# SeanNaren/deepspeech.pytorch

Hardware: NVIDIA H100
Metric: utterances/sec (train step, 161x1000 spectrogram) (higher is better)
Workload: dtype fp16-operands(rnn)+tf32(conv/fc)

## Files before the change

deepspeech.pytorch_b200/csrc/conv_tc.cu:

```cuda
#include "common.cuh"
#include "tc_common.cuh"

namespace ds2 {
int make_tmap_4d_f32(CUtensorMap* out, const float* base, const unsigned long long dims[4],
                     const unsigned long long strides_bytes[3], const unsigned int box[4]);
int make_tmap_nd_f32(CUtensorMap* out, const float* base, int rank, const unsigned long long* dims,
                     const unsigned long long* strides_bytes, const unsigned int* box);

namespace cv {
constexpr int CH = 32, KW = 11, NN = KW * CH;
constexpr int MP = 64, TO = MP - (KW - 1);
constexpr int A_BYTES = MP * 128;
constexpr int W_HALF = (NN / 2) * 128;
constexpr int STAGE_BYTES = A_BYTES + 2 * W_HALF;
constexpr int STAGES = 3;
constexpr int OUT_LD = 33, OUT_FLOATS = TO * OUT_LD;
constexpr int THREADS = 384;
constexpr int PRODUCER_REGS = 40, MMA_REGS = 232;
constexpr int ORDER_BAR = 1, EPI_BAR = 3;
constexpr int SMEM_BYTES = 1024 + STAGES * STAGE_BYTES + 2 * OUT_FLOATS * 4 + 256;
}

__device__ __forceinline__ void tma_load_4d_w(void* dst, const CUtensorMap* m, uint64_t* bar, int c0, int c1, int c2,
                                              int c3) {
  asm volatile(
      "{\n\t.reg .pred pe;\n\telect.sync _|pe, 0xffffffff;\n\t"
      "@pe cp.async.bulk.tensor.4d.shared::cluster.global.tile.mbarrier::complete_tx::bytes [%0], [%1, {%3, %4, %5, %6}], [%2];\n\t}"
      ::"r"(tc::smem_u32(dst)), "l"(reinterpret_cast<uint64_t>(m)), "r"(tc::smem_u32(bar)), "r"(c0), "r"(c1), "r"(c2),
        "r"(c3)
      : "memory");
}
__device__ __forceinline__ void tma_load_5d_w(void* dst, const CUtensorMap* m, uint64_t* bar, int c0, int c1, int c2,
                                              int c3, int c4) {
  asm volatile(
      "{\n\t.reg .pred pe;\n\telect.sync _|pe, 0xffffffff;\n\t"
      "@pe cp.async.bulk.tensor.5d.shared::cluster.global.tile.mbarrier::complete_tx::bytes [%0], [%1, {%3, %4, %5, %6, %7}], [%2];\n\t}"
      ::"r"(tc::smem_u32(dst)), "l"(reinterpret_cast<uint64_t>(m)), "r"(tc::smem_u32(bar)), "r"(c0), "r"(c1), "r"(c2),
        "r"(c3), "r"(c4)
      : "memory");
}

struct ConvTcParams {
  CUtensorMap tmA;
  CUtensorMap tmW;
  int B, T, R_in;
  int ntt;
  ConvRows rows[2];
  int tiles0, tiles;
  int row_mul, row_step, w_step, out_row_mul;
  float* out;
  size_t ob, oc, orow;
  const float* bias;
  const int32_t* out_len;
  double* stat_sums;
  double* piv_sums;
};

struct ConvTile {
  int t0, d, b, cls, j_lo, nj;
};
__device__ __forceinline__ ConvTile conv_tile(const ConvTcParams& p, int u) {
  ConvTile t;
  t.cls = u >= p.tiles0;
  if (t.cls) u -= p.tiles0;
  const ConvRows& rc = p.rows[t.cls];
  t.t0 = (u % p.ntt) * cv::TO;
  u /= p.ntt;
  t.d = u % rc.R_out;
  t.b = u / rc.R_out;
  int j_lo = 0, j_hi = rc.J;
  const int r0 = p.row_mul * t.d + rc.row_off;
  while (j_lo < j_hi && (r0 + j_lo * p.row_step < 0 || r0 + j_lo * p.row_step >= p.R_in)) ++j_lo;
  while (j_hi > j_lo && (r0 + (j_hi - 1) * p.row_step < 0 || r0 + (j_hi - 1) * p.row_step >= p.R_in)) --j_hi;
  t.j_lo = j_lo;
  t.nj = j_hi - j_lo;
  return t;
}

__device__ __forceinline__ void named_bar_sync(int id, int threads) {
  asm volatile("bar.sync %0, %1;" ::"r"(id), "r"(threads) : "memory");
}
__device__ __forceinline__ void named_bar_arrive(int id, int threads) {
  asm volatile("bar.arrive %0, %1;" ::"r"(id), "r"(threads) : "memory");
}

__global__ void __launch_bounds__(cv::THREADS, 1) conv_tc_kernel(const __grid_constant__ ConvTcParams p) {
  using namespace cv;
  using namespace tc;
  extern __shared__ uint8_t smem_raw[];
  uint8_t* smem = reinterpret_cast<uint8_t*>((reinterpret_cast<uintptr_t>(smem_raw) + 1023) & ~(uintptr_t)1023);
  float* out_s0 = reinterpret_cast<float*>(smem + STAGES * STAGE_BYTES);
  uint64_t* full = reinterpret_cast<uint64_t*>(out_s0 + 2 * OUT_FLOATS);
  uint64_t* empty = full + STAGES;

  const int warp = threadIdx.x / 32, lane = threadIdx.x % 32;

  if (warp == 0 && lane == 0) {
    tma_prefetch_desc(&p.tmA);
    tma_prefetch_desc(&p.tmW);
    for (int i = 0; i < STAGES; ++i) { mbar_init(&full[i], 1); mbar_init(&empty[i], 1); }
    fence_barrier_init();
  }
  __syncthreads();

  if (warp < 4) {
    setmaxnreg_dec<PRODUCER_REGS>();
    if (warp == 0) {
      int g = 0;
      for (int u = blockIdx.x; u < p.tiles; u += gridDim.x) {
        const ConvTile t = conv_tile(p, u);
        const ConvRows& rc = p.rows[t.cls];
        for (int jj = 0; jj < t.nj; ++jj, ++g) {
          const int j = t.j_lo + jj;
          const int r = p.row_mul * t.d + rc.row_off + j * p.row_step;
          const int wi = rc.w_off + j * p.w_step;
          const int s = g % STAGES;
          mbar_wait(&empty[s], ((g / STAGES) & 1) ^ 1);
          mbar_arrive_expect_tx_w(&full[s], (uint32_t)STAGE_BYTES);
          uint8_t* st = smem + s * STAGE_BYTES;
          tma_load_4d_w(st, &p.tmA, &full[s], 0, t.t0 - 5, r, t.b);
          tma_load_3d_w(st + A_BYTES, &p.tmW, &full[s], 0, 0, wi);
          tma_load_3d_w(st + A_BYTES + W_HALF, &p.tmW, &full[s], 0, NN / 2, wi);
        }
      }
    }
    return;
  }

  setmaxnreg_inc<MMA_REGS>();
  const int wg = warp / 4 - 1, w = warp % 4;
  const bool leader = (threadIdx.x & 127) == 0;
  float* out_s = out_s0 + wg * OUT_FLOATS;
  int g = 0;
  int i = 0;
  for (int u = blockIdx.x; u < p.tiles; u += gridDim.x, ++i) {
    const ConvTile t = conv_tile(p, u);
    if ((i & 1) != wg) {
      g += t.nj;
      continue;
    }
    if (i > 0) named_bar_sync(ORDER_BAR + wg, 256);
    float acc[NN / 2];
#pragma unroll
    for (int k = 0; k < NN / 2; ++k) acc[k] = 0.f;
    for (int jj = 0; jj < t.nj; ++jj, ++g) {
      const int s = g % STAGES;
      mbar_wait(&full[s], (g / STAGES) & 1);
      const uint64_t ad = smem_desc_sw128(smem_u32(smem + s * STAGE_BYTES));
      const uint64_t bd = smem_desc_sw128(smem_u32(smem + s * STAGE_BYTES + A_BYTES));
      wg_fence();
#pragma unroll
      for (int k = 0; k < 4; ++k) {
#pragma unroll
        for (int h = 0; h < 2; ++h)
          Wgmma<NN / 2, false>::mma(acc + (NN / 4) * h, ad + (uint64_t)(2 * k),
                                    bd + (uint64_t)(W_HALF / 16 * h + 2 * k), 1u);
      }
      wg_commit();
      wg_wait<1>();
      if (jj > 0 && leader) mbar_arrive(&empty[(g - 1) % STAGES]);
    }
    if (u + (int)gridDim.x < p.tiles) named_bar_arrive(ORDER_BAR + (wg ^ 1), 256);
    wg_wait<0>();
    if (t.nj > 0 && leader) mbar_arrive(&empty[(g - 1) % STAGES]);

    named_bar_sync(EPI_BAR + wg, 128);
#pragma unroll
    for (int kw = 0; kw < KW; ++kw) {
#pragma unroll
      for (int ib = 4 * kw; ib < 4 * kw + 4; ++ib) {
#pragma unroll
        for (int e = 0; e < 4; ++e) {
          const int pl = 16 * w + (lane >> 2) + 8 * (e >> 1);
          const int co = 8 * (ib % 4) + 2 * (lane & 3) + (e & 1);
          const int to = pl - kw;
          if (to >= 0 && to < TO) {
            float* o = out_s + to * OUT_LD + co;
            *o = (kw == 0 ? 0.f : *o) + acc[4 * ib + e];
          }
        }
      }
      named_bar_sync(EPI_BAR + wg, 128);
    }

    const int L = p.out_len ? p.out_len[t.b] : p.T;
    const int orow_idx = p.out_row_mul * t.d + p.rows[t.cls].out_row_off;
    for (int cc = 0; cc < 8; ++cc) {
      const int c = w * 8 + cc;
      const float bv = p.bias ? p.bias[c] : 0.f;
      float* op = p.out + (size_t)t.b * p.ob + (size_t)c * p.oc + (size_t)orow_idx * p.orow;
      float s1 = 0.f, s2 = 0.f, e1 = 0.f, e2 = 0.f;
      for (int to = lane; to < TO; to += 32) {
        const int tt = t.t0 + to;
        if (tt < p.T) {
          const float val = (tt < L) ? out_s[to * OUT_LD + c] + bv : 0.f;
          op[tt] = val;
          s1 += val;
          s2 = fmaf(val, val, s2);
          const float dv = val - bv;
          e1 += dv;
          e2 = fmaf(dv, dv, e2);
        }
      }
      if (p.stat_sums) {
        s1 = warp_sum(s1);
        s2 = warp_sum(s2);
        if (lane == 0) {
          atomicAdd(&p.stat_sums[c], (double)s1);
          atomicAdd(&p.stat_sums[CH + c], (double)s2);
        }
      }
      if (p.piv_sums) {
        e1 = warp_sum(e1);
        e2 = warp_sum(e2);
        if (lane == 0) {
          atomicAdd(&p.piv_sums[c], (double)e1);
          atomicAdd(&p.piv_sums[CH + c], (double)e2);
        }
      }
    }
  }
}

__global__ void pack_conv2_tc_fwd_kernel(const float* __restrict__ w2, float* __restrict__ wn) {
  int i = blockIdx.x * blockDim.x + threadIdx.x, n = 21 * cv::NN * 32;
  if (i >= n) return;
  int ci = i % 32, nn = (i / 32) % cv::NN, kh = i / (32 * cv::NN);
  int kw = nn / 32, co = nn % 32;
  wn[i] = w2[(((size_t)co * 32 + ci) * 21 + kh) * 11 + kw];
}
__global__ void pack_conv2_tc_bwd_kernel(const float* __restrict__ w2, float* __restrict__ wd) {
  int i = blockIdx.x * blockDim.x + threadIdx.x, n = 21 * cv::NN * 32;
  if (i >= n) return;
  int co = i % 32, nn = (i / 32) % cv::NN, kh = i / (32 * cv::NN);
  int kwi = nn / 32, ci = nn % 32;
  wd[i] = w2[(((size_t)co * 32 + ci) * 21 + kh) * 11 + (10 - kwi)];
}

__global__ void nchw_to_cl_kernel(int R, int T, const float* __restrict__ in, float* __restrict__ out) {
  __shared__ float tile[32][33];
  const int b = blockIdx.z, r = blockIdx.y, t0 = blockIdx.x * 32;
  for (int c = threadIdx.y; c < 32; c += 8) {
    int t = t0 + threadIdx.x;
    tile[c][threadIdx.x] = (t < T) ? in[(((size_t)b * 32 + c) * R + r) * T + t] : 0.f;
  }
  __syncthreads();
  for (int j = threadIdx.y; j < 32; j += 8) {
    int t = t0 + j;
    if (t < T) out[(((size_t)b * R + r) * T + t) * 32 + threadIdx.x] = tile[threadIdx.x][j];
  }
}

int nchw_to_cl(int B, int R, int T, const float* in, float* out, cudaStream_t st) {
  DS2_LAUNCH(nchw_to_cl_kernel, dim3(cdiv(T, 32), R, B), dim3(32, 8), 0, st, R, T, in, out);
  return DS2_OK;
}

int pack_conv2_tc(const float* w2, float* wn_fwd, float* wd_bwd, cudaStream_t st) {
  const int n = 21 * cv::NN * 32;
  if (wn_fwd) DS2_LAUNCH(pack_conv2_tc_fwd_kernel, cdiv(n, 256), 256, 0, st, w2, wn_fwd);
  if (wd_bwd) DS2_LAUNCH(pack_conv2_tc_bwd_kernel, cdiv(n, 256), 256, 0, st, w2, wd_bwd);
  return DS2_OK;
}

static int make_tmap_cl(CUtensorMap* out, const float* base, int T, int R, int B);

int conv_tc_run(const float* in_cl, int B, int T, int R_in, const float* taps, int n_taps, int row_mul, int row_step,
                int w_step, int out_row_mul, const ConvRows* rows, int n_classes, float* out, size_t ob, size_t oc,
                size_t orow, const float* bias, const int32_t* out_len, double* stat_sums, double* piv_sums,
                cudaStream_t st) {
  ConvTcParams p{};
  int rc = make_tmap_cl(&p.tmA, in_cl, T, R_in, B);
  if (rc) return rc;
  rc = make_tmap_3d(&p.tmW, taps, 32, cv::NN, n_taps, 32, (size_t)32 * cv::NN, 32, cv::NN / 2, 1);
  if (rc) return rc;
  p.B = B; p.T = T; p.R_in = R_in; p.ntt = cdiv(T, cv::TO);
  p.tiles = 0;
  for (int c = 0; c < n_classes; ++c) {
    p.rows[c] = rows[c];
    p.tiles += p.ntt * rows[c].R_out * B;
    if (c == 0) p.tiles0 = p.tiles;
  }
  p.row_mul = row_mul; p.row_step = row_step; p.w_step = w_step; p.out_row_mul = out_row_mul;
  p.out = out; p.ob = ob; p.oc = oc; p.orow = orow;
  p.bias = bias; p.out_len = out_len; p.stat_sums = stat_sums; p.piv_sums = piv_sums;
  static DeviceOnce attr_once;
  if (attr_once.first()) {
    DS2_CHECK_CUDA(cudaFuncSetAttribute(conv_tc_kernel, cudaFuncAttributeMaxDynamicSharedMemorySize, cv::SMEM_BYTES));
    attr_once.done();
  }
  const int grid = p.tiles < device_sm_count() ? p.tiles : device_sm_count();
  DS2_LAUNCH(conv_tc_kernel, grid, cv::THREADS, cv::SMEM_BYTES, st, p);
  return DS2_OK;
}

namespace wg {
constexpr int KT = 32;
constexpr int KH = 21;
constexpr int KH_PER = 2;
constexpr int GROUPS = 6;
constexpr int A_BYTES = KH_PER * 32 * 128;
constexpr int B_BYTES = cv::NN * 128;
constexpr int STAGE_BYTES = A_BYTES + B_BYTES;
constexpr int STAGES = 3;
constexpr int THREADS = 384;
constexpr int SMEM_BYTES = 1024 + STAGES * STAGE_BYTES + 256;
}

struct WgradParams {
  CUtensorMap tmDz;
  CUtensorMap tmS4;
  CUtensorMap tmS2;
  CUtensorMap tmS1;
  int B, T, slices;
  float* part;
};
__constant__ int KW_OF_BLOCK[11] = {1, 0, 5, 4, 3, 2, 9, 8, 7, 6, 10};

__global__ void shift_copies_kernel(size_t rows, int T, const float* __restrict__ a1, float* __restrict__ a1r) {
  const int Tp = T + 4;
  size_t i = (size_t)blockIdx.x * blockDim.x + threadIdx.x, n = rows * Tp, stride = (size_t)gridDim.x * blockDim.x;
  for (; i < n; i += stride) {
    const int t = (int)(i % Tp);
    const float* src = a1 + (i / Tp) * T;
#pragma unroll
    for (int sft = 0; sft <= 3; ++sft) {
      const int ts = t - sft;
      a1r[(size_t)sft * n + i] = (ts >= 0 && ts < T) ? src[ts] : 0.f;
    }
  }
}

__global__ void __launch_bounds__(wg::THREADS, 1) conv2_wgrad_tc_kernel(const __grid_constant__ WgradParams p) {
  using namespace wg;
  using namespace tc;
  extern __shared__ uint8_t smem_raw[];
  uint8_t* smem = reinterpret_cast<uint8_t*>((reinterpret_cast<uintptr_t>(smem_raw) + 1023) & ~(uintptr_t)1023);
  uint64_t* full = reinterpret_cast<uint64_t*>(smem + STAGES * STAGE_BYTES);
  uint64_t* empty = full + STAGES;
  const int warp = threadIdx.x / 32, lane = threadIdx.x % 32;
  const int parity = blockIdx.x / GROUPS, kh0 = parity + 2 * KH_PER * (blockIdx.x % GROUPS);
  if (kh0 >= KH) return;
  const int nkh = min(KH_PER, (KH - 1 - kh0) / 2 + 1);
  const int nr = (DS2_CONV1_D - parity + 1) / 2;
  const int pairs = p.B * nr;
  const int per = (pairs + (int)gridDim.y - 1) / (int)gridDim.y;
  const int p0 = blockIdx.y * per, p1 = min(pairs, p0 + per);
  const int nkt = (p.T + KT - 1) / KT;
  auto row_active = [&](int r) {
    const int d_hi = (r + 10 - kh0) / 2, d_lo = (r + 10 - (kh0 + 2 * (nkh - 1))) / 2;
    return d_hi >= 0 && d_lo < DS2_CONV2_D;
  };

  if (warp == 0 && lane == 0) {
    tma_prefetch_desc(&p.tmDz);
    tma_prefetch_desc(&p.tmS4);
    for (int i = 0; i < STAGES; ++i) { mbar_init(&full[i], 1); mbar_init(&empty[i], 2); }
    fence_barrier_init();
  }
  __syncthreads();

  int nchunks = 0;
  for (int pi = p0; pi < p1; ++pi)
    if (row_active(2 * (pi % nr) + parity)) nchunks += nkt;

  if (warp == 0) {
    int s = 0;
    uint32_t ph = 0;
    for (int pi = p0; pi < p1; ++pi) {
      const int b = pi / nr, r = 2 * (pi % nr) + parity;
      if (!row_active(r)) continue;
      for (int kt = 0; kt < nkt; ++kt) {
        mbar_wait(&empty[s], ph ^ 1);
        mbar_arrive_expect_tx_w(&full[s], (uint32_t)(nkh * 32 * 128 + cv::NN * 128));
        uint8_t* st = smem + s * STAGE_BYTES;
        for (int i = 0; i < nkh; ++i)
          tma_load_4d_w(st + i * 4096, &p.tmDz, &full[s], kt * KT, (r + 10 - kh0) / 2 - i, 0, b);
        uint8_t* nb = st + A_BYTES;
        tma_load_5d_w(nb, &p.tmS2, &full[s], kt * KT - 4, r, 0, b, 0);
        tma_load_5d_w(nb + 2 * 4096, &p.tmS4, &full[s], kt * KT, r, 0, b, 0);
        tma_load_5d_w(nb + 6 * 4096, &p.tmS4, &full[s], kt * KT + 4, r, 0, b, 0);
        tma_load_5d_w(nb + 10 * 4096, &p.tmS1, &full[s], kt * KT + 8, r, 0, b, 3);
        if (++s == STAGES) { s = 0; ph ^= 1; }
      }
    }
  } else if (warp >= 4) {
    const int wg = warp / 4 - 1;
    float acc[cv::NN / 4];
#pragma unroll
    for (int i = 0; i < cv::NN / 4; ++i) acc[i] = 0.f;
    int s = 0;
    uint32_t ph = 0;
    for (int c = 0; c < nchunks; ++c) {
      mbar_wait(&full[s], ph);
      const uint64_t ad = smem_desc_sw128(smem_u32(smem + s * STAGE_BYTES));
      const uint64_t bd = smem_desc_sw128(smem_u32(smem + s * STAGE_BYTES + A_BYTES + wg * cv::W_HALF));
      wg_fence();
#pragma unroll
      for (int k = 0; k < 4; ++k) Wgmma<cv::NN / 2, false>::mma(acc, ad + (uint64_t)(2 * k), bd + (uint64_t)(2 * k), 1u);
      wg_release(&empty[s]);
      if (++s == STAGES) { s = 0; ph ^= 1; }
    }
    const int w = warp % 4;
    float* tile = p.part + ((size_t)blockIdx.x * gridDim.y + blockIdx.y) * 64 * cv::NN;
#pragma unroll
    for (int i = 0; i < cv::NN / 16; ++i) {
#pragma unroll
      for (int hh = 0; hh < 2; ++hh) {
        const int m = 16 * w + (lane >> 2) + 8 * hh;
        const int n = cv::NN / 2 * wg + 8 * i + 2 * (lane & 3);
        *reinterpret_cast<float2*>(tile + (size_t)m * cv::NN + n) = make_float2(acc[4 * i + 2 * hh], acc[4 * i + 2 * hh + 1]);
      }
    }
  }
}

__global__ void conv2_wgrad_reduce_kernel(int slices, const float* __restrict__ part, float* __restrict__ dw2) {
  using namespace wg;
  const int idx = blockIdx.x * blockDim.x + threadIdx.x;
  if (idx >= 32 * 32 * KH * cv::KW) return;
  const int kw = idx % cv::KW, kh = (idx / cv::KW) % KH, ci = (idx / (cv::KW * KH)) % 32, co = idx / (cv::KW * KH * 32);
  const int parity = kh & 1, q = (kh - parity) / 2, x = parity * GROUPS + q / KH_PER, m = 32 * (q % KH_PER) + co;
  int blk = 0;
  while (KW_OF_BLOCK[blk] != kw) ++blk;
  const float* src = part + (size_t)x * slices * 64 * cv::NN + (size_t)m * cv::NN + blk * 32 + ci;
  float s = 0.f;
  for (int y = 0; y < slices; ++y) s += src[(size_t)y * 64 * cv::NN];
  dw2[idx] = s;
}

int conv2_wgrad_tc(const float* dz2, const float* a1, float* a1_shifted , float* part,
                   int B, int T, float* dw2, cudaStream_t st) {
  if (T % 4 != 0) return 1;
  WgradParams p{};
  {
    const size_t rows = (size_t)B * 32 * 81;
    DS2_LAUNCH(shift_copies_kernel, device_sm_count() * 8, 256, 0, st, rows, T, a1, a1_shifted);
    const unsigned long long Tq = (unsigned long long)T + 4;
    unsigned long long dims[5] = {Tq, 81ull, 32ull, (unsigned long long)B, 4ull};
    unsigned long long str[4] = {Tq * 4, 81ull * Tq * 4, 32ull * 81 * Tq * 4, (unsigned long long)rows * Tq * 4};
    unsigned int box[5] = {32u, 1u, 32u, 1u, 4u};
    int rc = make_tmap_nd_f32(&p.tmS4, a1_shifted, 5, dims, str, box);
    if (rc) return rc;
    box[4] = 2u;
    rc = make_tmap_nd_f32(&p.tmS2, a1_shifted, 5, dims, str, box);
    if (rc) return rc;
    box[4] = 1u;
    rc = make_tmap_nd_f32(&p.tmS1, a1_shifted, 5, dims, str, box);
    if (rc) return rc;
  }
  {
    unsigned long long dims[4] = {(unsigned long long)T, 41ull, 32ull, (unsigned long long)B};
    unsigned long long str[3] = {(unsigned long long)T * 4, (unsigned long long)41 * T * 4, (unsigned long long)32 * 41 * T * 4};
    unsigned int box[4] = {32u, 1u, 32u, 1u};
    int rc = make_tmap_4d_f32(&p.tmDz, dz2, dims, str, box);
    if (rc) return rc;
  }
  p.B = B; p.T = T; p.slices = 12; p.part = part;
  static DeviceOnce attr_once;
  if (attr_once.first()) {
    DS2_CHECK_CUDA(cudaFuncSetAttribute(conv2_wgrad_tc_kernel, cudaFuncAttributeMaxDynamicSharedMemorySize, wg::SMEM_BYTES));
    attr_once.done();
  }
  DS2_LAUNCH(conv2_wgrad_tc_kernel, dim3(2 * wg::GROUPS, p.slices), wg::THREADS, wg::SMEM_BYTES, st, p);
  DS2_LAUNCH(conv2_wgrad_reduce_kernel, cdiv(32 * 32 * wg::KH * cv::KW, 256), 256, 0, st, p.slices, part, dw2);
  return DS2_OK;
}

namespace w1 {
constexpr int KT = 32;
constexpr int DI = 4, RJ = 8;
constexpr int NROWS = 12 * RJ;
constexpr int CLASSES = 6;
constexpr int A_BYTES = 32 * DI * 128;
constexpr int B_BYTES = NROWS * 128;
constexpr int STAGE_BYTES = A_BYTES + B_BYTES;
constexpr int STAGES = 6;
constexpr int THREADS = 384;
constexpr int SMEM_BYTES = 1024 + STAGES * STAGE_BYTES + 256;
}
__constant__ int KW1_OF_GROUP[12] = {5, 6, 3, 4, 1, 2, -1, 0, 9, 10, 7, 8};

struct Wgrad1Params {
  CUtensorMap tmDz;
  CUtensorMap tmX8;
  CUtensorMap tmX4;
  int B, Tp;
  float* part;
};

__global__ void conv1_shift_copies_kernel(int B, int T, int Tp, const float* __restrict__ x, float* __restrict__ xs) {
  const int U = Tp + 4;
  const size_t rows = (size_t)B * DS2_NUM_FREQ, n = rows * U, total = 8 * n;
  for (size_t i = (size_t)blockIdx.x * blockDim.x + threadIdx.x; i < total; i += (size_t)gridDim.x * blockDim.x) {
    const int up = (int)(i % U);
    const size_t row = (i / U) % rows;
    const int sq = (int)(i / n), q = sq & 1, sft = sq >> 1;
    const int u = up - sft, tx = 2 * u + q;
    xs[i] = (u >= 0 && tx < T) ? x[row * T + tx] : 0.f;
  }
}

__global__ void __launch_bounds__(w1::THREADS, 1) conv1_wgrad_tc_kernel(const __grid_constant__ Wgrad1Params p) {
  using namespace w1;
  using namespace tc;
  extern __shared__ uint8_t smem_raw[];
  uint8_t* smem = reinterpret_cast<uint8_t*>((reinterpret_cast<uintptr_t>(smem_raw) + 1023) & ~(uintptr_t)1023);
  uint64_t* full = reinterpret_cast<uint64_t*>(smem + STAGES * STAGE_BYTES);
  uint64_t* empty = full + STAGES;
  const int warp = threadIdx.x / 32, lane = threadIdx.x % 32;
  const int cls = blockIdx.x;
  const int ndb = (DS2_CONV1_D + DI - 1) / DI;
  const int pairs = p.B * ndb;
  const int per = (pairs + (int)gridDim.y - 1) / (int)gridDim.y;
  const int p0 = blockIdx.y * per, p1 = min(pairs, p0 + per);
  const int nkt = (p.Tp + KT - 1) / KT;
  auto block_active = [&](int db) {
    const int r0 = 2 * DI * db - 20 + RJ * cls;
    return r0 + RJ - 1 >= 0 && r0 < DS2_NUM_FREQ;
  };

  if (warp == 0 && lane == 0) {
    tma_prefetch_desc(&p.tmDz);
    tma_prefetch_desc(&p.tmX8);
    tma_prefetch_desc(&p.tmX4);
    for (int i = 0; i < STAGES; ++i) { mbar_init(&full[i], 1); mbar_init(&empty[i], 2); }
    fence_barrier_init();
  }
  __syncthreads();

  int nchunks = 0;
  for (int pi = p0; pi < p1; ++pi)
    if (block_active(pi % ndb)) nchunks += nkt;

  if (warp == 0) {
    int s = 0;
    uint32_t ph = 0;
    for (int pi = p0; pi < p1; ++pi) {
      const int b = pi / ndb, db = pi % ndb;
      if (!block_active(db)) continue;
      const int d0 = DI * db, r0 = 2 * d0 - 20 + RJ * cls;
      for (int kt = 0; kt < nkt; ++kt) {
        mbar_wait(&empty[s], ph ^ 1);
        mbar_arrive_expect_tx_w(&full[s], (uint32_t)STAGE_BYTES);
        uint8_t* st = smem + s * STAGE_BYTES;
        tma_load_4d_w(st, &p.tmDz, &full[s], kt * KT, d0, 0, b);
        tma_load_5d_w(st + A_BYTES, &p.tmX8, &full[s], kt * KT, r0, b, 0, 0);
        tma_load_5d_w(st + A_BYTES + 64 * 128, &p.tmX4, &full[s], kt * KT + 4, r0, b, 0, 2);
        if (++s == STAGES) { s = 0; ph ^= 1; }
      }
    }
  } else if (warp >= 4) {
    const int wg = warp / 4 - 1;
    float acc[NROWS / 2];
#pragma unroll
    for (int i = 0; i < NROWS / 2; ++i) acc[i] = 0.f;
    int s = 0;
    uint32_t ph = 0;
    for (int c = 0; c < nchunks; ++c) {
      mbar_wait(&full[s], ph);
      const uint64_t ad = smem_desc_sw128(smem_u32(smem + s * STAGE_BYTES)) + (uint64_t)(512 * wg);
      const uint64_t bd = smem_desc_sw128(smem_u32(smem + s * STAGE_BYTES + A_BYTES));
      wg_fence();
#pragma unroll
      for (int k = 0; k < 4; ++k) Wgmma<NROWS, false>::mma(acc, ad + (uint64_t)(2 * k), bd + (uint64_t)(2 * k), 1u);
      wg_release(&empty[s]);
      if (++s == STAGES) { s = 0; ph ^= 1; }
    }
    const int w = warp % 4;
    float* tile = p.part + ((size_t)cls * gridDim.y + blockIdx.y) * 128 * NROWS;
#pragma unroll
    for (int i = 0; i < NROWS / 8; ++i) {
#pragma unroll
      for (int hh = 0; hh < 2; ++hh) {
        const int m = 64 * wg + 16 * w + (lane >> 2) + 8 * hh, n = 8 * i + 2 * (lane & 3);
        *reinterpret_cast<float2*>(tile + (size_t)m * NROWS + n) = make_float2(acc[4 * i + 2 * hh], acc[4 * i + 2 * hh + 1]);
      }
    }
  }
}

__global__ void conv1_wgrad_reduce_kernel(int slices, const float* __restrict__ part, float* __restrict__ dw1) {
  using namespace w1;
  const int idx = blockIdx.x * blockDim.x + threadIdx.x;
  if (idx >= 32 * 41 * 11) return;
  const int kw = idx % 11, kh = (idx / 11) % 41, co = idx / (11 * 41);
  int grp = 0;
  while (KW1_OF_GROUP[grp] != kw) ++grp;
  float s = 0.f;
  for (int cls = 0; cls < CLASSES; ++cls)
    for (int i = 0; i < DI; ++i) {
      const int j = kh - RJ * cls + 2 * i;
      if (j < 0 || j >= RJ) continue;
      const float* src = part + (size_t)cls * slices * 128 * NROWS + (size_t)(DI * co + i) * NROWS + grp * RJ + j;
      for (int y = 0; y < slices; ++y) s += src[(size_t)y * 128 * NROWS];
    }
  dw1[idx] = s;
}

size_t conv_wgrad_tc_partial_floats() {
  const size_t c2 = (size_t)2 * wg::GROUPS * 12 * 64 * cv::NN, c1 = (size_t)w1::CLASSES * 24 * 128 * w1::NROWS;
  return c2 > c1 ? c2 : c1;
}

int conv1_wgrad_tc(const float* dz1, const float* x, float* xs, float* part, int B, int T, int Tp, float* dw1,
                   cudaStream_t st) {
  if (Tp % 4 != 0) return 1;
  Wgrad1Params p{};
  const unsigned long long U = (unsigned long long)Tp + 4, F = DS2_NUM_FREQ;
  DS2_LAUNCH(conv1_shift_copies_kernel, device_sm_count() * 8, 256, 0, st, B, T, Tp, x, xs);
  {
    unsigned long long dims[5] = {U, F, (unsigned long long)B, 2ull, 4ull};
    unsigned long long str[4] = {U * 4, F * U * 4, (unsigned long long)B * F * U * 4, 2ull * B * F * U * 4};
    unsigned int box[5] = {32u, (unsigned int)w1::RJ, 1u, 2u, 4u};
    int rc = make_tmap_nd_f32(&p.tmX8, xs, 5, dims, str, box);
    if (rc) return rc;
    box[4] = 2u;
    rc = make_tmap_nd_f32(&p.tmX4, xs, 5, dims, str, box);
    if (rc) return rc;
  }
  {
    unsigned long long dims[4] = {(unsigned long long)Tp, (unsigned long long)DS2_CONV1_D, 32ull, (unsigned long long)B};
    unsigned long long str[3] = {(unsigned long long)Tp * 4, (unsigned long long)DS2_CONV1_D * Tp * 4,
                                 32ull * DS2_CONV1_D * Tp * 4};
    unsigned int box[4] = {32u, (unsigned int)w1::DI, 32u, 1u};
    int rc = make_tmap_4d_f32(&p.tmDz, dz1, dims, str, box);
    if (rc) return rc;
  }
  p.B = B; p.Tp = Tp; p.part = part;
  static DeviceOnce attr_once;
  if (attr_once.first()) {
    DS2_CHECK_CUDA(cudaFuncSetAttribute(conv1_wgrad_tc_kernel, cudaFuncAttributeMaxDynamicSharedMemorySize, w1::SMEM_BYTES));
    attr_once.done();
  }
  DS2_LAUNCH(conv1_wgrad_tc_kernel, dim3(w1::CLASSES, 24), w1::THREADS, w1::SMEM_BYTES, st, p);
  DS2_LAUNCH(conv1_wgrad_reduce_kernel, cdiv(32 * 41 * 11, 256), 256, 0, st, 24, part, dw1);
  return DS2_OK;
}

}

namespace ds2 {
int make_tmap_4d_f32(CUtensorMap* out, const float* base, const unsigned long long dims[4],
                     const unsigned long long strides_bytes[3], const unsigned int box[4]);
static int make_tmap_cl(CUtensorMap* out, const float* base, int T, int R, int B) {
  unsigned long long dims[4] = {32ull, (unsigned long long)T, (unsigned long long)R, (unsigned long long)B};
  unsigned long long str[3] = {128ull, (unsigned long long)T * 128ull, (unsigned long long)R * T * 128ull};
  unsigned int box[4] = {32u, (unsigned int)cv::MP, 1u, 1u};
  return make_tmap_4d_f32(out, base, dims, str, box);
}
}
```

Baseline: 655.4.

## Widen conv weight-gradient tiles and pipeline wgmma commits with deferred stage release

The conv2 weight-gradient kernel now covers four kernel-height taps per block instead of two, halving the group count. Each consumer warpgroup takes its own 64-row half of A and computes both N halves, with producer/consumer register rebalancing. The conv1 weight-gradient kernel processes two frequency classes per block, sharing the dz tile across both and halving its grid. Both kernels commit wgmma groups asynchronously and release the previous stage only after wait<1>, so MMAs overlap the next barrier wait. The cost is fewer blocks, which lowers SM occupancy, plus larger accumulators and more register pressure.

```diff
diff --git a/deepspeech.pytorch_b200/csrc/conv_tc.cu b/deepspeech.pytorch_b200/csrc/conv_tc.cu
--- a/deepspeech.pytorch_b200/csrc/conv_tc.cu
+++ b/deepspeech.pytorch_b200/csrc/conv_tc.cu
@@ -297,14 +297,17 @@
 namespace wg {
 constexpr int KT = 32;
 constexpr int KH = 21;
-constexpr int KH_PER = 2;
-constexpr int GROUPS = 6;
-constexpr int A_BYTES = KH_PER * 32 * 128;
+constexpr int KH_PER = 4;
+constexpr int GROUPS = 3;
+constexpr int M = KH_PER * 32;
+constexpr int A_BYTES = M * 128;
 constexpr int B_BYTES = cv::NN * 128;
 constexpr int STAGE_BYTES = A_BYTES + B_BYTES;
 constexpr int STAGES = 3;
+constexpr int SLICES = 12;
 constexpr int THREADS = 384;
 constexpr int SMEM_BYTES = 1024 + STAGES * STAGE_BYTES + 256;
+static_assert(2 * KH_PER * (GROUPS - 1) + 1 < KH && 2 * KH_PER * GROUPS >= KH, "every tap group of both parities has taps");
 }
 
 struct WgradParams {
@@ -312,7 +315,7 @@
   CUtensorMap tmS4;
   CUtensorMap tmS2;
   CUtensorMap tmS1;
-  int B, T, slices;
+  int B, T;
   float* part;
 };
 __constant__ int KW_OF_BLOCK[11] = {1, 0, 5, 4, 3, 2, 9, 8, 7, 6, 10};
@@ -340,11 +343,10 @@
   uint64_t* empty = full + STAGES;
   const int warp = threadIdx.x / 32, lane = threadIdx.x % 32;
   const int parity = blockIdx.x / GROUPS, kh0 = parity + 2 * KH_PER * (blockIdx.x % GROUPS);
-  if (kh0 >= KH) return;
   const int nkh = min(KH_PER, (KH - 1 - kh0) / 2 + 1);
   const int nr = (DS2_CONV1_D - parity + 1) / 2;
   const int pairs = p.B * nr;
-  const int per = (pairs + (int)gridDim.y - 1) / (int)gridDim.y;
+  const int per = (pairs + SLICES - 1) / SLICES;
   const int p0 = blockIdx.y * per, p1 = min(pairs, p0 + per);
   const int nkt = (p.T + KT - 1) / KT;
   auto row_active = [&](int r) {
@@ -364,58 +366,79 @@
   for (int pi = p0; pi < p1; ++pi)
     if (row_active(2 * (pi % nr) + parity)) nchunks += nkt;
 
-  if (warp == 0) {
-    int s = 0;
-    uint32_t ph = 0;
-    for (int pi = p0; pi < p1; ++pi) {
-      const int b = pi / nr, r = 2 * (pi % nr) + parity;
-      if (!row_active(r)) continue;
-      for (int kt = 0; kt < nkt; ++kt) {
-        mbar_wait(&empty[s], ph ^ 1);
-        mbar_arrive_expect_tx_w(&full[s], (uint32_t)(nkh * 32 * 128 + cv::NN * 128));
-        uint8_t* st = smem + s * STAGE_BYTES;
-        for (int i = 0; i < nkh; ++i)
-          tma_load_4d_w(st + i * 4096, &p.tmDz, &full[s], kt * KT, (r + 10 - kh0) / 2 - i, 0, b);
-        uint8_t* nb = st + A_BYTES;
-        tma_load_5d_w(nb, &p.tmS2, &full[s], kt * KT - 4, r, 0, b, 0);
-        tma_load_5d_w(nb + 2 * 4096, &p.tmS4, &full[s], kt * KT, r, 0, b, 0);
-        tma_load_5d_w(nb + 6 * 4096, &p.tmS4, &full[s], kt * KT + 4, r, 0, b, 0);
-        tma_load_5d_w(nb + 10 * 4096, &p.tmS1, &full[s], kt * KT + 8, r, 0, b, 3);
-        if (++s == STAGES) { s = 0; ph ^= 1; }
-      }
-    }
-  } else if (warp >= 4) {
-    const int wg = warp / 4 - 1;
-    float acc[cv::NN / 4];
-#pragma unroll
-    for (int i = 0; i < cv::NN / 4; ++i) acc[i] = 0.f;
-    int s = 0;
+  if (warp < 4) {
+    setmaxnreg_dec<cv::PRODUCER_REGS>();
+    if (warp == 0) {
+      int s = 0;
+      uint32_t ph = 0;
+      for (int pi = p0; pi < p1; ++pi) {
+        const int b = pi / nr, r = 2 * (pi % nr) + parity;
+        if (!row_active(r)) continue;
+        for (int kt = 0; kt < nkt; ++kt) {
+          mbar_wait(&empty[s], ph ^ 1);
+          mbar_arrive_expect_tx_w(&full[s], (uint32_t)(nkh * 32 * 128 + cv::NN * 128));
+          uint8_t* st = smem + s * STAGE_BYTES;
+          for (int i = 0; i < nkh; ++i)
+            tma_load_4d_w(st + i * 4096, &p.tmDz, &full[s], kt * KT, (r + 10 - kh0) / 2 - i, 0, b);
+          uint8_t* nb = st + A_BYTES;
+          tma_load_5d_w(nb, &p.tmS2, &full[s], kt * KT - 4, r, 0, b, 0);
+          tma_load_5d_w(nb + 2 * 4096, &p.tmS4, &full[s], kt * KT, r, 0, b, 0);
+          tma_load_5d_w(nb + 6 * 4096, &p.tmS4, &full[s], kt * KT + 4, r, 0, b, 0);
+          tma_load_5d_w(nb + 10 * 4096, &p.tmS1, &full[s], kt * KT + 8, r, 0, b, 3);
+          if (++s == STAGES) { s = 0; ph ^= 1; }
+        }
+      }
+    }
+    return;
+  }
+
+  setmaxnreg_inc<cv::MMA_REGS>();
+  const int wg = warp / 4 - 1;
+  const bool leader = (threadIdx.x & 127) == 0;
+  float acc[cv::NN / 2];
+#pragma unroll
+  for (int i = 0; i < cv::NN / 2; ++i) acc[i] = 0.f;
+  {
+    int s = 0, prev = 0;
     uint32_t ph = 0;
     for (int c = 0; c < nchunks; ++c) {
       mbar_wait(&full[s], ph);
-      const uint64_t ad = smem_desc_sw128(smem_u32(smem + s * STAGE_BYTES));
-      const uint64_t bd = smem_desc_sw128(smem_u32(smem + s * STAGE_BYTES + A_BYTES + wg * cv::W_HALF));
+      const uint64_t ad = smem_desc_sw128(smem_u32(smem + s * STAGE_BYTES)) + (uint64_t)(512 * wg);
+      const uint64_t bd = smem_desc_sw128(smem_u32(smem + s * STAGE_BYTES + A_BYTES));
       wg_fence();
 #pragma unroll
-      for (int k = 0; k < 4; ++k) Wgmma<cv::NN / 2, false>::mma(acc, ad + (uint64_t)(2 * k), bd + (uint64_t)(2 * k), 1u);
-      wg_release(&empty[s]);
+      for (int k = 0; k < 4; ++k) {
+#pragma unroll
+        for (int h = 0; h < 2; ++h)
+          Wgmma<cv::NN / 2, false>::mma(acc + (cv::NN / 4) * h, ad + (uint64_t)(2 * k),
+                                        bd + (uint64_t)(cv::W_HALF / 16 * h + 2 * k), 1u);
+      }
+      wg_commit();
+      wg_wait<1>();
+      if (c > 0 && leader) mbar_arrive(&empty[prev]);
+      prev = s;
       if (++s == STAGES) { s = 0; ph ^= 1; }
     }
+    wg_wait<0>();
+    if (nchunks > 0 && leader) mbar_arrive(&empty[prev]);
+  }
+
+  {
     const int w = warp % 4;
-    float* tile = p.part + ((size_t)blockIdx.x * gridDim.y + blockIdx.y) * 64 * cv::NN;
-#pragma unroll
-    for (int i = 0; i < cv::NN / 16; ++i) {
+    float* tile = p.part + ((size_t)blockIdx.x * SLICES + blockIdx.y) * M * cv::NN;
+#pragma unroll
+    for (int i = 0; i < cv::NN / 8; ++i) {
 #pragma unroll
       for (int hh = 0; hh < 2; ++hh) {
-        const int m = 16 * w + (lane >> 2) + 8 * hh;
-        const int n = cv::NN / 2 * wg + 8 * i + 2 * (lane & 3);
+        const int m = 64 * wg + 16 * w + (lane >> 2) + 8 * hh;
+        const int n = cv::NN / 2 * (i / (cv::NN / 16)) + 8 * (i % (cv::NN / 16)) + 2 * (lane & 3);
         *reinterpret_cast<float2*>(tile + (size_t)m * cv::NN + n) = make_float2(acc[4 * i + 2 * hh], acc[4 * i + 2 * hh + 1]);
       }
     }
   }
 }
 
-__global__ void conv2_wgrad_reduce_kernel(int slices, const float* __restrict__ part, float* __restrict__ dw2) {
+__global__ void conv2_wgrad_reduce_kernel(const float* __restrict__ part, float* __restrict__ dw2) {
   using namespace wg;
   const int idx = blockIdx.x * blockDim.x + threadIdx.x;
   if (idx >= 32 * 32 * KH * cv::KW) return;
@@ -423,9 +446,9 @@
   const int parity = kh & 1, q = (kh - parity) / 2, x = parity * GROUPS + q / KH_PER, m = 32 * (q % KH_PER) + co;
   int blk = 0;
   while (KW_OF_BLOCK[blk] != kw) ++blk;
-  const float* src = part + (size_t)x * slices * 64 * cv::NN + (size_t)m * cv::NN + blk * 32 + ci;
+  const float* src = part + (size_t)x * SLICES * M * cv::NN + (size_t)m * cv::NN + blk * 32 + ci;
   float s = 0.f;
-  for (int y = 0; y < slices; ++y) s += src[(size_t)y * 64 * cv::NN];
+  for (int y = 0; y < SLICES; ++y) s += src[(size_t)y * M * cv::NN];
   dw2[idx] = s;
 }
 
@@ -456,14 +479,14 @@
     int rc = make_tmap_4d_f32(&p.tmDz, dz2, dims, str, box);
     if (rc) return rc;
   }
-  p.B = B; p.T = T; p.slices = 12; p.part = part;
+  p.B = B; p.T = T; p.part = part;
   static DeviceOnce attr_once;
   if (attr_once.first()) {
     DS2_CHECK_CUDA(cudaFuncSetAttribute(conv2_wgrad_tc_kernel, cudaFuncAttributeMaxDynamicSharedMemorySize, wg::SMEM_BYTES));
     attr_once.done();
   }
-  DS2_LAUNCH(conv2_wgrad_tc_kernel, dim3(2 * wg::GROUPS, p.slices), wg::THREADS, wg::SMEM_BYTES, st, p);
-  DS2_LAUNCH(conv2_wgrad_reduce_kernel, cdiv(32 * 32 * wg::KH * cv::KW, 256), 256, 0, st, p.slices, part, dw2);
+  DS2_LAUNCH(conv2_wgrad_tc_kernel, dim3(2 * wg::GROUPS, wg::SLICES), wg::THREADS, wg::SMEM_BYTES, st, p);
+  DS2_LAUNCH(conv2_wgrad_reduce_kernel, cdiv(32 * 32 * wg::KH * cv::KW, 256), 256, 0, st, part, dw2);
   return DS2_OK;
 }
 
@@ -472,10 +495,12 @@
 constexpr int DI = 4, RJ = 8;
 constexpr int NROWS = 12 * RJ;
 constexpr int CLASSES = 6;
+constexpr int CPC = 2;
 constexpr int A_BYTES = 32 * DI * 128;
 constexpr int B_BYTES = NROWS * 128;
-constexpr int STAGE_BYTES = A_BYTES + B_BYTES;
-constexpr int STAGES = 6;
+constexpr int STAGE_BYTES = A_BYTES + CPC * B_BYTES;
+constexpr int STAGES = 5;
+constexpr int SLICES = 24;
 constexpr int THREADS = 384;
 constexpr int SMEM_BYTES = 1024 + STAGES * STAGE_BYTES + 256;
 }
@@ -509,15 +534,15 @@
   uint64_t* full = reinterpret_cast<uint64_t*>(smem + STAGES * STAGE_BYTES);
   uint64_t* empty = full + STAGES;
   const int warp = threadIdx.x / 32, lane = threadIdx.x % 32;
-  const int cls = blockIdx.x;
+  const int cls0 = CPC * blockIdx.x;
   const int ndb = (DS2_CONV1_D + DI - 1) / DI;
   const int pairs = p.B * ndb;
   const int per = (pairs + (int)gridDim.y - 1) / (int)gridDim.y;
   const int p0 = blockIdx.y * per, p1 = min(pairs, p0 + per);
   const int nkt = (p.Tp + KT - 1) / KT;
   auto block_active = [&](int db) {
-    const int r0 = 2 * DI * db - 20 + RJ * cls;
-    return r0 + RJ - 1 >= 0 && r0 < DS2_NUM_FREQ;
+    const int r0 = 2 * DI * db - 20 + RJ * cls0;
+    return r0 + CPC * RJ - 1 >= 0 && r0 < DS2_NUM_FREQ;
   };
 
   if (warp == 0 && lane == 0) {
@@ -539,23 +564,29 @@
     for (int pi = p0; pi < p1; ++pi) {
       const int b = pi / ndb, db = pi % ndb;
       if (!block_active(db)) continue;
-      const int d0 = DI * db, r0 = 2 * d0 - 20 + RJ * cls;
+      const int d0 = DI * db, r0 = 2 * d0 - 20 + RJ * cls0;
       for (int kt = 0; kt < nkt; ++kt) {
         mbar_wait(&empty[s], ph ^ 1);
         mbar_arrive_expect_tx_w(&full[s], (uint32_t)STAGE_BYTES);
         uint8_t* st = smem + s * STAGE_BYTES;
         tma_load_4d_w(st, &p.tmDz, &full[s], kt * KT, d0, 0, b);
-        tma_load_5d_w(st + A_BYTES, &p.tmX8, &full[s], kt * KT, r0, b, 0, 0);
-        tma_load_5d_w(st + A_BYTES + 64 * 128, &p.tmX4, &full[s], kt * KT + 4, r0, b, 0, 2);
+        for (int c = 0; c < CPC; ++c) {
+          uint8_t* bt = st + A_BYTES + c * B_BYTES;
+          tma_load_5d_w(bt, &p.tmX8, &full[s], kt * KT, r0 + RJ * c, b, 0, 0);
+          tma_load_5d_w(bt + 64 * 128, &p.tmX4, &full[s], kt * KT + 4, r0 + RJ * c, b, 0, 2);
+        }
         if (++s == STAGES) { s = 0; ph ^= 1; }
       }
     }
   } else if (warp >= 4) {
     const int wg = warp / 4 - 1;
-    float acc[NROWS / 2];
-#pragma unroll
-    for (int i = 0; i < NROWS / 2; ++i) acc[i] = 0.f;
-    int s = 0;
+    float acc[CPC][NROWS / 2];
+#pragma unroll
+    for (int c = 0; c < CPC; ++c)
+#pragma unroll
+      for (int i = 0; i < NROWS / 2; ++i) acc[c][i] = 0.f;
+    const bool leader = (threadIdx.x & 127) == 0;
+    int s = 0, prev = 0;
     uint32_t ph = 0;
     for (int c = 0; c < nchunks; ++c) {
       mbar_wait(&full[s], ph);
@@ -563,24 +594,37 @@
       const uint64_t bd = smem_desc_sw128(smem_u32(smem + s * STAGE_BYTES + A_BYTES));
       wg_fence();
 #pragma unroll
-      for (int k = 0; k < 4; ++k) Wgmma<NROWS, false>::mma(acc, ad + (uint64_t)(2 * k), bd + (uint64_t)(2 * k), 1u);
-      wg_release(&empty[s]);
+      for (int k = 0; k < 4; ++k) {
+#pragma unroll
+        for (int c = 0; c < CPC; ++c)
+          Wgmma<NROWS, false>::mma(acc[c], ad + (uint64_t)(2 * k), bd + (uint64_t)(B_BYTES / 16 * c + 2 * k), 1u);
+      }
+      wg_commit();
+      wg_wait<1>();
+      if (c > 0 && leader) mbar_arrive(&empty[prev]);
+      prev = s;
       if (++s == STAGES) { s = 0; ph ^= 1; }
     }
+    wg_wait<0>();
+    if (nchunks > 0 && leader) mbar_arrive(&empty[prev]);
     const int w = warp % 4;
-    float* tile = p.part + ((size_t)cls * gridDim.y + blockIdx.y) * 128 * NROWS;
-#pragma unroll
-    for (int i = 0; i < NROWS / 8; ++i) {
-#pragma unroll
-      for (int hh = 0; hh < 2; ++hh) {
-        const int m = 64 * wg + 16 * w + (lane >> 2) + 8 * hh, n = 8 * i + 2 * (lane & 3);
-        *reinterpret_cast<float2*>(tile + (size_t)m * NROWS + n) = make_float2(acc[4 * i + 2 * hh], acc[4 * i + 2 * hh + 1]);
-      }
-    }
-  }
-}
-
-__global__ void conv1_wgrad_reduce_kernel(int slices, const float* __restrict__ part, float* __restrict__ dw1) {
+#pragma unroll
+    for (int c = 0; c < CPC; ++c) {
+      float* tile = p.part + ((size_t)(cls0 + c) * SLICES + blockIdx.y) * 128 * NROWS;
+#pragma unroll
+      for (int i = 0; i < NROWS / 8; ++i) {
+#pragma unroll
+        for (int hh = 0; hh < 2; ++hh) {
+          const int m = 64 * wg + 16 * w + (lane >> 2) + 8 * hh, n = 8 * i + 2 * (lane & 3);
+          *reinterpret_cast<float2*>(tile + (size_t)m * NROWS + n) =
+              make_float2(acc[c][4 * i + 2 * hh], acc[c][4 * i + 2 * hh + 1]);
+        }
+      }
+    }
+  }
+}
+
+__global__ void conv1_wgrad_reduce_kernel(const float* __restrict__ part, float* __restrict__ dw1) {
   using namespace w1;
   const int idx = blockIdx.x * blockDim.x + threadIdx.x;
   if (idx >= 32 * 41 * 11) return;
@@ -592,14 +636,15 @@
     for (int i = 0; i < DI; ++i) {
       const int j = kh - RJ * cls + 2 * i;
       if (j < 0 || j >= RJ) continue;
-      const float* src = part + (size_t)cls * slices * 128 * NROWS + (size_t)(DI * co + i) * NROWS + grp * RJ + j;
-      for (int y = 0; y < slices; ++y) s += src[(size_t)y * 128 * NROWS];
+      const float* src = part + (size_t)cls * SLICES * 128 * NROWS + (size_t)(DI * co + i) * NROWS + grp * RJ + j;
+      for (int y = 0; y < SLICES; ++y) s += src[(size_t)y * 128 * NROWS];
     }
   dw1[idx] = s;
 }
 
 size_t conv_wgrad_tc_partial_floats() {
-  const size_t c2 = (size_t)2 * wg::GROUPS * 12 * 64 * cv::NN, c1 = (size_t)w1::CLASSES * 24 * 128 * w1::NROWS;
+  const size_t c2 = (size_t)2 * wg::GROUPS * wg::SLICES * wg::M * cv::NN;
+  const size_t c1 = (size_t)w1::CLASSES * w1::SLICES * 128 * w1::NROWS;
   return c2 > c1 ? c2 : c1;
 }
 
@@ -633,8 +678,8 @@
     DS2_CHECK_CUDA(cudaFuncSetAttribute(conv1_wgrad_tc_kernel, cudaFuncAttributeMaxDynamicSharedMemorySize, w1::SMEM_BYTES));
     attr_once.done();
   }
-  DS2_LAUNCH(conv1_wgrad_tc_kernel, dim3(w1::CLASSES, 24), w1::THREADS, w1::SMEM_BYTES, st, p);
-  DS2_LAUNCH(conv1_wgrad_reduce_kernel, cdiv(32 * 41 * 11, 256), 256, 0, st, 24, part, dw1);
+  DS2_LAUNCH(conv1_wgrad_tc_kernel, dim3(w1::CLASSES / w1::CPC, w1::SLICES), w1::THREADS, w1::SMEM_BYTES, st, p);
+  DS2_LAUNCH(conv1_wgrad_reduce_kernel, cdiv(32 * 41 * 11, 256), 256, 0, st, part, dw1);
   return DS2_OK;
 }
 
```

Result: faster. 666.6, median of 6 (+1.7%).
